# mynameisfiber/baton

Hardware: AMD Instinct MI355X
Metric: fed_local_samples_per_sec (higher is better)
Workload: dtype bf16; 1 GPU; model=resnet18, global_batch=8192, image=32x32x3, parallelism=federated-dp1 (FedAvg E=1), local_samples_per_round=16384, optimizer=sgd, hip_graph=True

## Files before the change

baton_amd/ops/csrc/bindings.cpp:

```cpp
#include <torch/extension.h>
#include <ATen/hip/HIPContext.h>

#include "launchers.h"
#include "wgrad_px_map.h"

namespace {

bool is_bf16(const at::Tensor& t) { return t.scalar_type() == at::kBFloat16; }

void check_compute(const at::Tensor& t, const char* name) {
  TORCH_CHECK(t.is_cuda(), name, " must be on GPU");
  TORCH_CHECK(t.is_contiguous(), name, " must be contiguous");
  TORCH_CHECK(t.scalar_type() == at::kFloat || t.scalar_type() == at::kBFloat16,
              name, " must be fp32 or bf16");
}

hipStream_t stream() { return at::hip::getCurrentHIPStream().stream(); }

void run_dense(const GemmProblem& p, const GemmPlan& pl, const void* A,
               const void* B, void* C, const float* bias, long long strideA = 0,
               long long strideB = 0, long long strideC = 0, int b_group = 1,
               GemmStrides gs = GemmStrides{0, 0, 0, 1, 0, 0, 0}) {
  if (pl.kind == GemmKind::G9) {
    TORCH_CHECK(launch_gemm_nt_g9(pl, A, B, C, bias, pl.m_main, p.N, p.K,
                                  (float)p.alpha, stream()),
                "gemm: G9 plan does not fit ", pl.m_main, "x", p.N, "x", p.K);
    if (pl.m_main == p.M) return;
    const GemmProblem r = gemm_remainder(p, pl);
    run_dense(r, plan_dense(r),
              (const at::BFloat16*)A + (long long)pl.m_main * p.K, B,
              (at::BFloat16*)C + (long long)pl.m_main * p.N, bias);
    return;
  }
  TORCH_CHECK(launch_gemm_2ph(pl, p, A, B, C, bias, strideA, strideB, strideC,
                              stream(), b_group, gs),
              "gemm: 2-phase plan does not fit ", p.M, "x", p.N, "x", p.K);
}

void run_slab(const GemmPlan& pl, const at::Tensor& A, const at::Tensor& B,
              at::Tensor& out, int M, int N, int K) {
  auto slabs = at::empty({(long long)pl.splits * M * N},
                         A.options().dtype(at::kFloat));
  TORCH_CHECK(launch_gemm_nt_slab(pl, A.data_ptr(), B.data_ptr(),
                                  slabs.data_ptr<float>(), out.data_ptr(),
                                  out.scalar_type() != at::kFloat, M, N, K,
                                  stream()),
              "gemm: slab plan does not fit ", M, "x", N, "x", K);
}

void run_splitk(const GemmPlan& pl, const at::Tensor& A, const at::Tensor& B,
                at::Tensor& out, int M, int N, int K) {
  TORCH_CHECK(launch_gemm_2ph_splitk(pl, is_bf16(A), A.data_ptr(), B.data_ptr(),
                                     out.data_ptr<float>(), M, N, K, stream()),
              "gemm: split-K plan does not fit ", M, "x", N, "x", K);
}

}


void sgd_step(at::Tensor p, at::Tensor g, at::Tensor m, double lr,
              double momentum, double weight_decay, bool zero_grad) {
  check_compute(p, "p");
  check_compute(g, "g");
  TORCH_CHECK(p.scalar_type() == g.scalar_type(), "p/g dtype mismatch");
  TORCH_CHECK(p.numel() == g.numel(), "p/g numel mismatch");
  float* mptr = nullptr;
  if (m.defined() && m.numel() > 0) {
    TORCH_CHECK(m.scalar_type() == at::kFloat && m.is_contiguous());
    TORCH_CHECK(m.numel() == p.numel());
    mptr = m.data_ptr<float>();
  }
  launch_sgd(is_bf16(p), p.data_ptr(), g.data_ptr(), mptr, p.numel(), (float)lr,
             (float)momentum, (float)weight_decay, zero_grad ? 1 : 0,
             stream());
}

void adam_step(at::Tensor p, at::Tensor g, at::Tensor m, at::Tensor v,
               double lr, double beta1, double beta2, double eps,
               double weight_decay, double bc1, double bc2, bool zero_grad) {
  check_compute(p, "p");
  check_compute(g, "g");
  TORCH_CHECK(m.scalar_type() == at::kFloat && v.scalar_type() == at::kFloat);
  TORCH_CHECK(p.numel() == g.numel() && p.numel() == m.numel() &&
              p.numel() == v.numel());
  launch_adam(is_bf16(p), p.data_ptr(), g.data_ptr(), m.data_ptr<float>(),
              v.data_ptr<float>(), p.numel(), (float)lr, (float)beta1,
              (float)beta2, (float)eps, (float)weight_decay,
// ... 464 lines not shown
      launch_conv_wgrad(is_bf16(x), dyt.data_ptr(), x.data_ptr(),
                        dw32.data_ptr(), N, H, W, Cin, Cout, (int)KH, (int)KW,
                        (int)stride, (int)pad, stream());
    }
  }
  if (out_f32 || x.scalar_type() == at::kFloat) return dw32;
  auto dw = at::empty({Cout, KH, KW, Cin}, x.options());
  launch_cast_copy(true, dw.data_ptr(), dw32.data_ptr<float>(), dw.numel(),
                   stream());
  return dw;
}


py::dict wgrad_px_map(int64_t N, int64_t H, int64_t W, int64_t step) {
  using namespace py::literals;
  TORCH_CHECK(wgpx::eligible(true, (int)N, (int)H, (int)W, 64, 64, 3, 3, 1, 1),
              "wgrad_px_map: shape not eligible");
  const wgpx::Geom g = wgpx::make_geom((int)H, (int)W);
  const long long p0 = step * wgpx::PXK;
  TORCH_CHECK(step >= 0 && p0 < N * H * W, "wgrad_px_map: step out of range");
  const int h0 = (int)((p0 / W) % H);
  const int passes = wgpx::passes_of((int)W);
  py::list stage, window, dy_rows;
  for (int i = 0; i < wgpx::PXK; ++i) dy_rows.append(py::none());
  for (int i = 0; i < g.slots; ++i) window.append(py::none());
  for (int c = 0; c < passes * wgpx::THREADS; ++c) {
    const wgpx::ChunkSrc cs = wgpx::chunk_src(g, c);
    const bool ok = cs.kind == 1 ||
                    (cs.kind == 2 && wgpx::x_row_valid(g, h0, cs.hrel));
    const long long px = ok ? p0 + cs.rel : -1;
    stage.append(py::make_tuple(c / wgpx::THREADS, c % wgpx::THREADS, 16 * c,
                                ok ? cs.kind : 0, px, cs.sub));
    const int row = c / wgpx::CPR;
    if (c % wgpx::CPR == 0 && row < wgpx::PXK) dy_rows[row] = cs.rel;
    if (c % wgpx::CPR == 0 && row >= wgpx::PXK && row < wgpx::PXK + g.slots &&
        ok)
      window[row - wgpx::PXK] = py::make_tuple(
          px / (H * W), (px / W) % H, px % W);
  }
  py::list kpix, a_addr, b_addr;
  for (int k = 0; k < wgpx::PXK; ++k)
    kpix.append(wgpx::lin_pixel((int)W, wgpx::kslot_lin(k)));
  for (int r = 0; r < 2; ++r) {
    py::list la;
    for (int l = 0; l < 64; ++l) la.append(wgpx::a_read_addr(l, r));
    a_addr.append(la);
  }
  for (int t = 0; t < 9; ++t) {
    py::list lt;
    for (int r = 0; r < 2; ++r) {
      py::list lb;
      for (int l = 0; l < 64; ++l)
        lb.append(wgpx::b_read_addr(g, l, r) +
                  wgpx::tap_off(g, t / 3, t % 3) * wgpx::ROWB);
      lt.append(lb);
    }
    b_addr.append(lt);
  }
  return py::dict(
      "row_bytes"_a = wgpx::ROWB, "dy_rows_base"_a = 0,
      "window_base"_a = wgpx::PXK * wgpx::ROWB, "pitch"_a = g.pitch,
      "window_rows"_a = g.wrows, "slots"_a = g.slots, "passes"_a = passes,
      "threads"_a = wgpx::THREADS, "buffer_bytes"_a = passes * wgpx::THREADS * 16,
      "claimed_conflict_degree"_a = 1, "stage"_a = stage, "window"_a = window,
      "dy_rows"_a = dy_rows, "kslot_pixel"_a = kpix, "a_addr"_a = a_addr,
      "b_addr"_a = b_addr);
}

bool wgrad_px_eligible(bool bf16, int64_t N, int64_t H, int64_t W, int64_t Cin,
                       int64_t Cout, int64_t KH, int64_t KW, int64_t stride,
                       int64_t pad) {
  return wgpx::eligible(bf16, (int)N, (int)H, (int)W, (int)Cin, (int)Cout,
                        (int)KH, (int)KW, (int)stride, (int)pad);
}

py::tuple wgrad_px_split(int64_t N, int64_t H, int64_t W, int64_t Cin,
                         int64_t Cout) {
  const long long steps = N * H * W / wgpx::PXK;
  const int sps = wgpx::steps_per_split(
      steps, (int)(Cin / wgpx::TILE) * (int)(Cout / wgpx::TILE));
  return py::make_tuple(steps, sps, (steps + sps - 1) / sps);
}


at::Tensor bmm_strided(at::Tensor A, at::Tensor B, c10::optional<at::Tensor> C_in,
                       int64_t layout, int64_t M, int64_t N, int64_t K,
                       int64_t nbatch, int64_t heads, int64_t b_group,
                       double alpha,
                       int64_t saO, int64_t saI, int64_t lda,
                       int64_t sbO, int64_t sbI, int64_t ldb,
                       int64_t scO, int64_t scI, int64_t ldc) {
  TORCH_CHECK(A.is_cuda() && B.is_cuda(), "bmm_strided: GPU tensors required");
  TORCH_CHECK(A.scalar_type() == B.scalar_type());
  TORCH_CHECK(A.scalar_type() == at::kFloat || A.scalar_type() == at::kBFloat16);
  at::Tensor C;
  if (C_in.has_value() && C_in->defined()) {
    C = *C_in;
    TORCH_CHECK(C.is_cuda() && C.scalar_type() == A.scalar_type());
  } else {
    C = at::empty({nbatch, M, N}, A.options());
    scO = (int64_t)heads * M * N;
    scI = (int64_t)M * N;
    ldc = N;
  }
  GemmStrides gs{lda, ldb, ldc, (int)heads, saI, sbI, scI};
  const GemmProblem p{is_bf16(A), false, (int)layout, (int)M, (int)N, (int)K,
                      false, false, alpha, 0.0, true, (int)nbatch,
                      gs.heads > 1 || gs.lda || gs.ldb || gs.ldc};
  run_dense(p, plan_dense(p), A.data_ptr(), B.data_ptr(), C.data_ptr(), nullptr,
            saO, sbO, scO, (int)b_group, gs);
  return C;
}


at::Tensor gemm_batched(at::Tensor A, at::Tensor B, int64_t layout,
                        bool out_f32, double alpha, int64_t b_group) {
  check_compute(A, "A");
  check_compute(B, "B");
  TORCH_CHECK(A.dim() == 3 && B.dim() == 3, "gemm_batched wants 3-D tensors");
  TORCH_CHECK(A.size(0) == B.size(0) * b_group, "batch/group mismatch");
  int nb = A.size(0);
  int M, N, K;
  if (layout == 0) {
    M = A.size(1); K = A.size(2); N = B.size(1);
    TORCH_CHECK(B.size(2) == K);
  } else if (layout == 1) {
    M = A.size(1); K = A.size(2); N = B.size(2);
    TORCH_CHECK(B.size(1) == K);
  } else {
    K = A.size(1); M = A.size(2); N = B.size(2);
    TORCH_CHECK(B.size(1) == K);
  }
  auto C = at::empty({nb, M, N},
                     A.options().dtype(out_f32 ? at::kFloat : A.scalar_type()));
  const GemmProblem p{is_bf16(A), out_f32, (int)layout, M, N, K, false, false,
                      alpha, 0.0, true, nb, false};
  run_dense(p, plan_dense(p), A.data_ptr(), B.data_ptr(), C.data_ptr(), nullptr,
            (long long)A.size(1) * A.size(2), (long long)B.size(1) * B.size(2),
            (long long)M * N, (int)b_group);
  return C;
}

at::Tensor softmax_fwd(at::Tensor x, double scale, int64_t causal_seq) {
  check_compute(x, "x");
  int C = x.size(-1);
  long long R = x.numel() / C;
  auto y = at::empty_like(x);
  launch_softmax_fwd(is_bf16(x), x.data_ptr(), y.data_ptr(), R, C,
                     (float)scale, (int)causal_seq, stream());
  return y;
}

at::Tensor softmax_bwd(at::Tensor y, at::Tensor dy, double scale) {
  check_compute(y, "y");
  check_compute(dy, "dy");
  int C = y.size(-1);
  long long R = y.numel() / C;
  auto dx = at::empty_like(y);
  launch_softmax_bwd(is_bf16(y), y.data_ptr(), dy.data_ptr(), dx.data_ptr(), R,
                     C, (float)scale, stream());
  return dx;
}



std::vector<at::Tensor> rms_fwd(at::Tensor x, at::Tensor w, double eps) {
// ... 178 lines not shown
      "flash_bwd_dq: unsupported head_dim ", DH);
  TORCH_CHECK(
      launch_flash_bwd_dkv(q.data_ptr(), k.data_ptr(), v.data_ptr(),
                           dout.data_ptr(), lse.data_ptr<float>(),
                           delta.data_ptr<float>(), dk.data_ptr(),
                           dv.data_ptr(), B, S, H, G, DH, scale, causal, qs,
                           ks, vs, dos, dks, dvs, stream()),
      "flash_bwd_dkv: unsupported head_dim ", DH);
}

PYBIND11_MODULE(TORCH_EXTENSION_NAME, m) {
  m.def("flash_fwd", &flash_fwd);
  m.def("flash_bwd", &flash_bwd);
  m.def("rms_add_fwd", &rms_add_fwd);
  m.def("rms_bwd_plus", &rms_bwd_plus);
  m.def("sgd_step", &sgd_step, "fused SGD step", py::arg("p"), py::arg("g"),
        py::arg("m"), py::arg("lr"), py::arg("momentum"),
        py::arg("weight_decay"), py::arg("zero_grad") = false);
  m.def("adam_step", &adam_step, "fused Adam step", py::arg("p"), py::arg("g"),
        py::arg("m"), py::arg("v"), py::arg("lr"), py::arg("beta1"),
        py::arg("beta2"), py::arg("eps"), py::arg("weight_decay"),
        py::arg("bc1"), py::arg("bc2"), py::arg("zero_grad") = false);
  m.def("scale_cast", &scale_cast);
  m.def("cast_copy", &cast_copy);
  m.def("axpby", &axpby);
  m.def("bmm_strided", &bmm_strided, py::arg("A"), py::arg("B"),
        py::arg("C_in") = py::none(), py::arg("layout") = 0,
        py::arg("M") = 0, py::arg("N") = 0, py::arg("K") = 0,
        py::arg("nbatch") = 1, py::arg("heads") = 1,
        py::arg("b_group") = 1, py::arg("alpha") = 1.0,
        py::arg("saO") = 0, py::arg("saI") = 0, py::arg("lda") = 0,
        py::arg("sbO") = 0, py::arg("sbI") = 0, py::arg("ldb") = 0,
        py::arg("scO") = 0, py::arg("scI") = 0, py::arg("ldc") = 0);
  m.def("colsum", &colsum);
  m.def("mse_fwd", &mse_fwd);
  m.def("mse_bwd", &mse_bwd);
  m.def("ce_fwd", &ce_fwd);
  m.def("ce_bwd", &ce_bwd);
  m.def("ln_fwd", &ln_fwd);
  m.def("ln_bwd", &ln_bwd);
  m.def("ln_add_fwd", &ln_add_fwd);
  m.def("ln_bwd_plus", &ln_bwd_plus);
  m.def("bn_fwd_train", &bn_fwd_train, py::arg("x"), py::arg("gamma"),
        py::arg("beta"), py::arg("running_mean"), py::arg("running_var"),
        py::arg("momentum"), py::arg("eps"), py::arg("relu"),
        py::arg("res") = py::none());
  m.def("bn_fwd_eval", &bn_fwd_eval);
  m.def("bn_bwd", &bn_bwd, py::arg("x"), py::arg("dy"), py::arg("y_post"),
        py::arg("mean"), py::arg("rstd"), py::arg("gamma"), py::arg("relu"),
        py::arg("want_dres") = false);
  m.def("relu_fwd", &relu_fwd);
  m.def("relu_bwd", &relu_bwd);
  m.def("add_relu_fwd", &add_relu_fwd);
  m.def("add_scaled_fwd", &add_scaled_fwd);
  m.def("scale_fwd", &scale_fwd);
  m.def("gelu_fwd", &gelu_fwd);
  m.def("gelu_bwd", &gelu_bwd);
  m.def("gemm", &gemm, py::arg("A"), py::arg("B"), py::arg("layout"),
        py::arg("bias") = py::none(), py::arg("relu") = false,
        py::arg("out_f32") = false, py::arg("alpha") = 1.0,
        py::arg("beta") = 0.0, py::arg("C_in") = py::none(),
        py::arg("direct") = false);
  m.def("gemm_plan", &gemm_plan, py::arg("M"), py::arg("N"), py::arg("K"),
        py::arg("layout") = 0, py::arg("bf16") = true,
        py::arg("out_f32") = false, py::arg("has_bias") = false,
        py::arg("relu") = false, py::arg("alpha") = 1.0, py::arg("beta") = 0.0,
        py::arg("direct") = false, py::arg("nbatch") = 1,
        py::arg("strided") = false, py::arg("batched") = false);
  m.def("gemm_batched", &gemm_batched, py::arg("A"), py::arg("B"),
        py::arg("layout"), py::arg("out_f32") = false, py::arg("alpha") = 1.0,
        py::arg("b_group") = 1);
  m.def("softmax_fwd", &softmax_fwd, py::arg("x"), py::arg("scale") = 1.0,
        py::arg("causal_seq") = 0);
  m.def("softmax_bwd", &softmax_bwd);
  m.def("rms_fwd", &rms_fwd);
  m.def("rms_bwd", &rms_bwd);
  m.def("rope", &rope, py::arg("x"), py::arg("cos_t"), py::arg("sin_t"),
        py::arg("inverse") = false);
  m.def("silu_mul_fwd", &silu_mul_fwd);
  m.def("silu_mul_bwd", &silu_mul_bwd);
  m.def("conv_fwd", &conv_fwd);
  m.def("conv_dgrad", &conv_dgrad);
  m.def("conv_wgrad", &conv_wgrad);
  m.def("wgrad_px_map", &wgrad_px_map, py::arg("N"), py::arg("H"),
        py::arg("W"), py::arg("step"));
  m.def("wgrad_px_eligible", &wgrad_px_eligible);
  m.def("wgrad_px_split", &wgrad_px_split);
}
```

baton_amd/ops/csrc/conv.hip:

```cpp
#include "common.h"

constexpr int CBK = 32;
constexpr int CFRAG = 16;

struct ConvShape {
  int N, H, W, Cin, Cout, KH, KW, stride, pad, HO, WO, swz;
};



template <int ROWS>
DEVINL void stage_glds_rows(bf16* __restrict__ lds, const bf16* __restrict__ src,
                            long long ld, long long row0, int k0) {
  const int t = threadIdx.x;
  const int w = t >> 6;
  constexpr int TOTAL = ROWS * 4;
#pragma unroll
  for (int p = 0; p * kBlock < TOTAL; ++p) {
    const int idx = p * kBlock + t;
    if (idx >= TOTAL) break;
    const int row = idx >> 2;
    const int psl = idx & 3;
    const int lsl = psl ^ ((row >> 2) & 3);
    auto g = (const __attribute__((address_space(1))) unsigned int*)(
        src + (row0 + row) * ld + k0 + lsl * 8);
    auto l = (__attribute__((address_space(3))) unsigned int*)(
        lds + (long long)(p * kBlock + w * 64) * 8);
    __builtin_amdgcn_global_load_lds(g, l, 16, 0, 0);
  }
}

template <typename T, int ROWS, bool FAST>
struct FwdAStager {
  static constexpr int ELEMS = 16 / (int)sizeof(T);
  static constexpr int TPR = CBK / ELEMS;
  static constexpr int RPP = kBlock / TPR;
  static constexpr int PASSES = ROWS / RPP;
  int kc;
  int row[PASSES];
  int n[PASSES], ho[PASSES], wo[PASSES];
  bool ok[PASSES];
  int ci, kw, kh;
  int k_generic;
  int m0_;
  bool full_;

  DEVINL void init(const ConvShape& sh, int m0, int Mtot) {
    m0_ = m0;
    full_ = (m0 + ROWS <= Mtot);
    kc = (threadIdx.x % TPR) * ELEMS;
#pragma unroll
    for (int p = 0; p < PASSES; ++p) {
      row[p] = p * RPP + threadIdx.x / TPR;
      const int m = m0 + row[p];
      wo[p] = m % sh.WO;
      const int t = m / sh.WO;
      ho[p] = t % sh.HO;
      n[p] = t / sh.HO;
      ok[p] = m < Mtot;
    }
    ci = kc;
    kw = 0;
    kh = 0;
    k_generic = kc;
  }

  DEVINL void stage(T* __restrict__ lds, const T* __restrict__ x,
                    const ConvShape& sh, int Ktot) {
    using VT = typename VecTraits<T>::VecT;
    if constexpr (sizeof(T) == 2 && FAST) {
      if (sh.KH == 1 && sh.stride == 1 && full_ && (sh.Cin % 8) == 0) {
        stage_glds_rows<ROWS>((bf16*)lds, (const bf16*)x, sh.Cin,
                              (long long)m0_, ci - kc);
        ci += CBK;
        if (ci >= sh.Cin) {
          ci -= sh.Cin;
          if (++kw == sh.KW) { kw = 0; ++kh; }
        }
        return;
      }
    }
#pragma unroll
    for (int p = 0; p < PASSES; ++p) {
// ... 68 lines not shown
                    ? w[(long long)(n0 + row) * ld + k0 + kc + j]
                    : (T)0.f;
    }
    *reinterpret_cast<VT*>(&lds[lds_off<T>(row, kc)]) = v;
  }
}

template <typename T, int ROWS, bool FAST>
struct DgradAStager {
  static constexpr int ELEMS = 16 / (int)sizeof(T);
  static constexpr int TPR = CBK / ELEMS;
  static constexpr int RPP = kBlock / TPR;
  static constexpr int PASSES = ROWS / RPP;
  int kc;
  int n[PASSES], hq[PASSES], wq[PASSES];
  bool ok[PASSES];
  int co, kw, kh;
  int k_generic;

  DEVINL void init(const ConvShape& sh, int m0, int Mtot) {
    kc = (threadIdx.x % TPR) * ELEMS;
#pragma unroll
    for (int p = 0; p < PASSES; ++p) {
      const int q = m0 + p * RPP + threadIdx.x / TPR;
      wq[p] = q % sh.W;
      const int t = q / sh.W;
      hq[p] = t % sh.H;
      n[p] = t / sh.H;
      ok[p] = q < Mtot;
    }
    co = kc;
    kw = 0;
    kh = 0;
    k_generic = kc;
  }

  DEVINL void stage(T* __restrict__ lds, const T* __restrict__ dy,
                    const ConvShape& sh, int Ktot) {
    using VT = typename VecTraits<T>::VecT;
#pragma unroll
    for (int p = 0; p < PASSES; ++p) {
      VT v;
      T* vp = reinterpret_cast<T*>(&v);
#pragma unroll
      for (int j = 0; j < ELEMS; ++j) vp[j] = (T)0.f;
      if (FAST) {
        if (ok[p]) {
          const int hnum = hq[p] + sh.pad - kh, wnum = wq[p] + sh.pad - kw;
          if (hnum >= 0 && wnum >= 0 && hnum % sh.stride == 0 &&
              wnum % sh.stride == 0) {
            const int ho = hnum / sh.stride, wo = wnum / sh.stride;
            if (ho < sh.HO && wo < sh.WO)
              v = *reinterpret_cast<const VT*>(
                  &dy[(((long long)n[p] * sh.HO + ho) * sh.WO + wo) * sh.Cout + co]);
          }
        }
      } else if (ok[p]) {
#pragma unroll
        for (int j = 0; j < ELEMS; ++j) {
          const int k = k_generic + j;
          if (k < Ktot) {
            const int coj = k % sh.Cout, tap = k / sh.Cout;
            const int kwj = tap % sh.KW, khj = tap / sh.KW;
            const int hnum = hq[p] + sh.pad - khj, wnum = wq[p] + sh.pad - kwj;
            if (hnum >= 0 && wnum >= 0 && hnum % sh.stride == 0 &&
                wnum % sh.stride == 0) {
              const int ho = hnum / sh.stride, wo = wnum / sh.stride;
              if (ho < sh.HO && wo < sh.WO)
                vp[j] = dy[(((long long)n[p] * sh.HO + ho) * sh.WO + wo) * sh.Cout + coj];
            }
          }
        }
      }
      *reinterpret_cast<VT*>(&lds[lds_off<T>(p * RPP + threadIdx.x / TPR, kc)]) = v;
    }
    if (FAST) {
      co += CBK;
      if (co >= sh.Cout) {
        co -= sh.Cout;
        if (++kw == sh.KW) { kw = 0; ++kh; }
      }
    } else {
      k_generic += CBK;
    }
  }
};

template <typename T, int ROWS>
struct WgradBStager {
  static constexpr int ELEMS = 16 / (int)sizeof(T);
  static constexpr int VPK = ROWS / ELEMS;
  static constexpr int TOTAL = CBK * VPK;
  static constexpr int PASSES = (TOTAL + kBlock - 1) / kBlock;
  int k_in_tile[PASSES], rr[PASSES], r_local[PASSES];
  int ci[PASSES], kw[PASSES], kh[PASSES];
  bool active[PASSES], one_tap[PASSES], r_ok[PASSES];
  int wo[PASSES], ho[PASSES], nn[PASSES];
  bool p_ok[PASSES];

  DEVINL void init(const ConvShape& sh, int n0, long long p0, long long p_limit,
                   int Rtot) {
#pragma unroll
    for (int p = 0; p < PASSES; ++p) {
      const int idx = p * kBlock + threadIdx.x;
      active[p] = idx < TOTAL;
      k_in_tile[p] = idx / VPK;
      r_local[p] = (idx % VPK) * ELEMS;
      rr[p] = n0 + r_local[p];
      r_ok[p] = rr[p] < Rtot;
      ci[p] = r_ok[p] ? rr[p] % sh.Cin : 0;
      const int tap = r_ok[p] ? rr[p] / sh.Cin : 0;
      kw[p] = tap % sh.KW;
      kh[p] = tap / sh.KW;
      one_tap[p] = (rr[p] / sh.Cin) == ((rr[p] + ELEMS - 1) / sh.Cin);
      const long long px = p0 + k_in_tile[p];
      p_ok[p] = px < p_limit;
      wo[p] = (int)(px % sh.WO);
      const long long t = px / sh.WO;
      ho[p] = (int)(t % sh.HO);
      nn[p] = (int)(t / sh.HO);
    }
  }

  DEVINL void stage(T* __restrict__ lds, const T* __restrict__ x,
                    const ConvShape& sh) {
    using VT = typename VecTraits<T>::VecT;
#pragma unroll
    for (int p = 0; p < PASSES; ++p) {
      if (!active[p]) continue;
      VT v;
      T* vp = reinterpret_cast<T*>(&v);
#pragma unroll
      for (int j = 0; j < ELEMS; ++j) vp[j] = (T)0.f;
      if (p_ok[p] && r_ok[p]) {
        if (one_tap[p]) {
          const int hi = ho[p] * sh.stride - sh.pad + kh[p];
          const int wi = wo[p] * sh.stride - sh.pad + kw[p];
          if (hi >= 0 && hi < sh.H && wi >= 0 && wi < sh.W)
            v = *reinterpret_cast<const VT*>(
                &x[(((long long)nn[p] * sh.H + hi) * sh.W + wi) * sh.Cin + ci[p]]);
        } else {
#pragma unroll
          for (int j = 0; j < ELEMS; ++j) {
            const int rj = rr[p] + j;
            const int cij = rj % sh.Cin, tapj = rj / sh.Cin;
            const int kwj = tapj % sh.KW, khj = tapj / sh.KW;
            const int hi = ho[p] * sh.stride - sh.pad + khj;
            const int wi = wo[p] * sh.stride - sh.pad + kwj;
            if (hi >= 0 && hi < sh.H && wi >= 0 && wi < sh.W)
              vp[j] = x[(((long long)nn[p] * sh.H + hi) * sh.W + wi) * sh.Cin + cij];
          }
        }
      }
#pragma unroll
      for (int j = 0; j < ELEMS; ++j)
        lds[lds_off<T>(r_local[p] + j, k_in_tile[p])] = vp[j];
      wo[p] += CBK;
      while (wo[p] >= sh.WO) {
        wo[p] -= sh.WO;
        if (++ho[p] == sh.HO) { ho[p] = 0; ++nn[p]; }
      }
    }
  }

  DEVINL void set_p_ok(long long p0, long long p_limit) {
#pragma unroll
// ... 75 lines not shown
  FwdAStager<T, BM, FAST> sa;
  sa.init(sh, m0, Mtot);
  sa.stage(a_lds[0], x, sh, Ktot);
  stage_fwd_B<T, BN>(b_lds[0], w, n0, 0, Ntot, Ktot, Ktot);
  __syncthreads();
  for (int kt = 0; kt < nk; ++kt) {
    const int cur = kt & 1;
    if (kt + 1 < nk) {
      sa.stage(a_lds[cur ^ 1], x, sh, Ktot);
      stage_fwd_B<T, BN>(b_lds[cur ^ 1], w, n0, (kt + 1) * CBK, Ntot, Ktot, Ktot);
    }
    conv_mma<T, MF, NF>(a_lds[cur], b_lds[cur], acc, lane, wm0, wn0);
    __syncthreads();
  }
  const int col_in_frag = lane & 15, row_base = (lane >> 4) * 4;
#pragma unroll
  for (int mf = 0; mf < MF; ++mf)
#pragma unroll
    for (int nf = 0; nf < NF; ++nf)
#pragma unroll
      for (int r = 0; r < 4; ++r) {
        int row = m0 + wm0 + mf * CFRAG + row_base + r;
        int col = n0 + wn0 + nf * CFRAG + col_in_frag;
        if (row < Mtot && col < Ntot)
          y[(long long)row * Ntot + col] = (T)acc[mf][nf][r];
      }
}

template <typename T, int BM, int BN, int WAVES_M, int WAVES_N, bool FAST>
__global__ __launch_bounds__(kBlock) void conv_dgrad_kernel(
    const T* __restrict__ dy, const T* __restrict__ w_t, T* __restrict__ dx,
    ConvShape sh) {
  constexpr int WM = BM / WAVES_M, WN = BN / WAVES_N;
  constexpr int MF = WM / CFRAG, NF = WN / CFRAG;
  __shared__ T a_lds[2][BM * lds_row_elems<T>()];
  __shared__ T b_lds[2][BN * lds_row_elems<T>()];
  const int Mtot = sh.N * sh.H * sh.W;
  const int Ntot = sh.Cin;
  const int Ktot = sh.KH * sh.KW * sh.Cout;
  int t_n, t_m;
  {
    const int nwg = gridDim.x * gridDim.y;
    int bid = blockIdx.y * gridDim.x + blockIdx.x;
    if (sh.swz && nwg >= 64) {
      const int q = nwg >> 3, r = nwg & 7;
      const int xcd = bid & 7, idx = bid >> 3;
      bid = (xcd < r ? xcd * (q + 1) : r * (q + 1) + (xcd - r) * q) + idx;
    }
    t_n = bid % gridDim.x;
    t_m = bid / gridDim.x;
  }
  const int m0 = t_m * BM, n0 = t_n * BN;
  const int lane = threadIdx.x & (kWave - 1);
  const int wid = threadIdx.x / kWave;
  const int wm0 = (wid / WAVES_N) * WM, wn0 = (wid % WAVES_N) * WN;
  f32x4 acc[MF][NF] = {};
  const int nk = (Ktot + CBK - 1) / CBK;
  DgradAStager<T, BM, FAST> sa;
  sa.init(sh, m0, Mtot);
  sa.stage(a_lds[0], dy, sh, Ktot);
  stage_fwd_B<T, BN>(b_lds[0], w_t, n0, 0, Ntot, Ktot, Ktot);
  __syncthreads();
  for (int kt = 0; kt < nk; ++kt) {
    const int cur = kt & 1;
    if (kt + 1 < nk) {
      sa.stage(a_lds[cur ^ 1], dy, sh, Ktot);
      stage_fwd_B<T, BN>(b_lds[cur ^ 1], w_t, n0, (kt + 1) * CBK, Ntot, Ktot, Ktot);
    }
    conv_mma<T, MF, NF>(a_lds[cur], b_lds[cur], acc, lane, wm0, wn0);
    __syncthreads();
  }
  const int col_in_frag = lane & 15, row_base = (lane >> 4) * 4;
#pragma unroll
  for (int mf = 0; mf < MF; ++mf)
#pragma unroll
    for (int nf = 0; nf < NF; ++nf)
#pragma unroll
      for (int r = 0; r < 4; ++r) {
        int row = m0 + wm0 + mf * CFRAG + row_base + r;
        int col = n0 + wn0 + nf * CFRAG + col_in_frag;
        if (row < Mtot && col < Ntot)
          dx[(long long)row * Ntot + col] = (T)acc[mf][nf][r];
      }
}

template <typename T, int BM, int BN, int WAVES_M, int WAVES_N>
__global__ __launch_bounds__(kBlock) void conv_wgrad_kernel(
    const T* __restrict__ dy_t, const T* __restrict__ x, float* __restrict__ dw,
    ConvShape sh, long long p_chunk) {
  constexpr int WM = BM / WAVES_M, WN = BN / WAVES_N;
  constexpr int MF = WM / CFRAG, NF = WN / CFRAG;
  __shared__ T a_lds[2][BM * lds_row_elems<T>()];
  __shared__ T b_lds[2][BN * lds_row_elems<T>()];
  const int Mtot = sh.Cout;
  const int Ntot = sh.KH * sh.KW * sh.Cin;
  const long long Ptot = (long long)sh.N * sh.HO * sh.WO;
  const long long p_begin = (long long)blockIdx.z * p_chunk;
  const long long p_end = min(p_begin + p_chunk, Ptot);
  const int m0 = blockIdx.y * BM, n0 = blockIdx.x * BN;
  const int lane = threadIdx.x & (kWave - 1);
  const int wid = threadIdx.x / kWave;
  const int wm0 = (wid / WAVES_N) * WM, wn0 = (wid % WAVES_N) * WN;
  f32x4 acc[MF][NF] = {};
  const long long nk = (p_end - p_begin + CBK - 1) / CBK;
  if (nk <= 0) return;
  WgradBStager<T, BN> sb;
  sb.init(sh, n0, p_begin, p_end, Ntot);
  stage_fwd_B<T, BM>(a_lds[0], dy_t, m0, (int)p_begin, Mtot, (int)p_end, Ptot);
  sb.stage(b_lds[0], x, sh);
  __syncthreads();
  for (long long kt = 0; kt < nk; ++kt) {
    const int cur = (int)(kt & 1);
    if (kt + 1 < nk) {
      stage_fwd_B<T, BM>(a_lds[cur ^ 1], dy_t, m0,
                         (int)(p_begin + (kt + 1) * CBK), Mtot, (int)p_end,
                         Ptot);
      sb.set_p_ok(p_begin + (kt + 1) * CBK, p_end);
      sb.stage(b_lds[cur ^ 1], x, sh);
    }
    conv_mma<T, MF, NF>(a_lds[cur], b_lds[cur], acc, lane, wm0, wn0);
    __syncthreads();
  }
  const int col_in_frag = lane & 15, row_base = (lane >> 4) * 4;
#pragma unroll
  for (int mf = 0; mf < MF; ++mf)
#pragma unroll
    for (int nf = 0; nf < NF; ++nf)
#pragma unroll
      for (int r = 0; r < 4; ++r) {
        int row = m0 + wm0 + mf * CFRAG + row_base + r;
        int col = n0 + wn0 + nf * CFRAG + col_in_frag;
        if (row < Mtot && col < Ntot) {
          if (gridDim.z == 1)
            dw[(long long)row * Ntot + col] = acc[mf][nf][r];
          else
            atomicAdd(&dw[(long long)row * Ntot + col], acc[mf][nf][r]);
        }
      }
}

#define INST_CONV(T)                                                        \
  template __global__ void conv_fwd_kernel<T, 128, 128, 2, 2, true>(        \
      const T*, const T*, T*, ConvShape);                                   \
  template __global__ void conv_fwd_kernel<T, 128, 128, 2, 2, false>(       \
      const T*, const T*, T*, ConvShape);                                   \
  template __global__ void conv_fwd_kernel<T, 128, 64, 4, 1, true>(         \
      const T*, const T*, T*, ConvShape);                                   \
  template __global__ void conv_fwd_kernel<T, 128, 64, 4, 1, false>(        \
      const T*, const T*, T*, ConvShape);                                   \
  template __global__ void conv_dgrad_kernel<T, 128, 128, 2, 2, true>(      \
      const T*, const T*, T*, ConvShape);                                   \
  template __global__ void conv_dgrad_kernel<T, 128, 128, 2, 2, false>(     \
      const T*, const T*, T*, ConvShape);                                   \
  template __global__ void conv_dgrad_kernel<T, 128, 64, 4, 1, true>(       \
      const T*, const T*, T*, ConvShape);                                   \
  template __global__ void conv_dgrad_kernel<T, 128, 64, 4, 1, false>(      \
      const T*, const T*, T*, ConvShape);                                   \
  template __global__ void conv_wgrad_kernel<T, 128, 128, 2, 2>(            \
      const T*, const T*, float*, ConvShape, long long);                    \
  template __global__ void conv_wgrad_kernel<T, 64, 128, 1, 4>(             \
      const T*, const T*, float*, ConvShape, long long);

INST_CONV(bf16)
INST_CONV(float)

#include "launchers.h"

static ConvShape make_shape(int N, int H, int W, int Cin, int Cout, int KH,
                            int KW, int stride, int pad) {
  ConvShape sh;
  sh.N = N; sh.H = H; sh.W = W; sh.Cin = Cin; sh.Cout = Cout;
  sh.KH = KH; sh.KW = KW; sh.stride = stride; sh.pad = pad;
  sh.HO = (H + 2 * pad - KH) / stride + 1;
  sh.WO = (W + 2 * pad - KW) / stride + 1;
  long long act = (long long)N * H * W * Cin + (long long)N * sh.HO * sh.WO * Cout;
  sh.swz = act * 2 > (200LL << 20) ? 1 : 0;
  return sh;
}

void launch_conv_fwd(bool is_bf16, const void* x, const void* w, void* y,
                     int N, int H, int W, int Cin, int Cout, int KH, int KW,
                     int stride, int pad, hipStream_t s) {
  ConvShape sh = make_shape(N, H, W, Cin, Cout, KH, KW, stride, pad);
  long long M = (long long)N * sh.HO * sh.WO;
  const bool narrow = Cout <= 64;
  const bool fast = (Cin % CBK) == 0;
  const int BN_ = narrow ? 64 : 128;
  dim3 grid((Cout + BN_ - 1) / BN_, (M + 127) / 128);
  #define FWD(T, BM, BN, WM, WN, F)                                         \
    hipLaunchKernelGGL((conv_fwd_kernel<T, BM, BN, WM, WN, F>), grid,       \
                       dim3(kBlock), 0, s, (const T*)x, (const T*)w, (T*)y, sh)
  if (is_bf16) {
    if (narrow) { if (fast) FWD(bf16, 128, 64, 4, 1, true); else FWD(bf16, 128, 64, 4, 1, false); }
    else { if (fast) FWD(bf16, 128, 128, 2, 2, true); else FWD(bf16, 128, 128, 2, 2, false); }
  } else {
    if (narrow) { if (fast) FWD(float, 128, 64, 4, 1, true); else FWD(float, 128, 64, 4, 1, false); }
    else { if (fast) FWD(float, 128, 128, 2, 2, true); else FWD(float, 128, 128, 2, 2, false); }
  }
  #undef FWD
}

void launch_conv_dgrad(bool is_bf16, const void* dy, const void* w, void* dx,
                       int N, int H, int W, int Cin, int Cout, int KH, int KW,
                       int stride, int pad, hipStream_t s) {
  ConvShape sh = make_shape(N, H, W, Cin, Cout, KH, KW, stride, pad);
  long long M = (long long)N * H * W;
  const bool narrow = Cin <= 64;
  const bool fast = (Cout % CBK) == 0;
  const int BN_ = narrow ? 64 : 128;
  dim3 grid((Cin + BN_ - 1) / BN_, (M + 127) / 128);
  #define DG(T, BM, BN, WM, WN, F)                                          \
    hipLaunchKernelGGL((conv_dgrad_kernel<T, BM, BN, WM, WN, F>), grid,     \
                       dim3(kBlock), 0, s, (const T*)dy, (const T*)w, (T*)dx, sh)
  if (is_bf16) {
    if (narrow) { if (fast) DG(bf16, 128, 64, 4, 1, true); else DG(bf16, 128, 64, 4, 1, false); }
    else { if (fast) DG(bf16, 128, 128, 2, 2, true); else DG(bf16, 128, 128, 2, 2, false); }
  } else {
    if (narrow) { if (fast) DG(float, 128, 64, 4, 1, true); else DG(float, 128, 64, 4, 1, false); }
    else { if (fast) DG(float, 128, 128, 2, 2, true); else DG(float, 128, 128, 2, 2, false); }
  }
  #undef DG
}

void launch_conv_wgrad(bool is_bf16, const void* dy, const void* x, void* dw,
                       int N, int H, int W, int Cin, int Cout, int KH, int KW,
                       int stride, int pad, hipStream_t s) {
  ConvShape sh = make_shape(N, H, W, Cin, Cout, KH, KW, stride, pad);
  int Ntot = KH * KW * Cin;
  const bool narrow_m = Cout <= 64;
  const int BM_ = narrow_m ? 64 : 128;
  int tiles_x = (Ntot + 127) / 128;
  int tiles_y = (Cout + BM_ - 1) / BM_;
  long long Ptot = (long long)N * sh.HO * sh.WO;
  int target = 512 / (tiles_x * tiles_y);
  if (target < 1) target = 1;
  long long max_splits = (Ptot + CBK - 1) / CBK;
  int splits = (int)(max_splits < target ? max_splits : target);
  long long p_chunk = ((Ptot + splits - 1) / splits + CBK - 1) / CBK * CBK;
  splits = (int)((Ptot + p_chunk - 1) / p_chunk);
  dim3 grid(tiles_x, tiles_y, splits);
  #define WG(T, BM, BN, WM, WN)                                             \
    hipLaunchKernelGGL((conv_wgrad_kernel<T, BM, BN, WM, WN>), grid,        \
                       dim3(kBlock), 0, s, (const T*)dy, (const T*)x,       \
                       (float*)dw, sh, p_chunk)
  if (is_bf16) { if (narrow_m) WG(bf16, 64, 128, 1, 4); else WG(bf16, 128, 128, 2, 2); }
  else { if (narrow_m) WG(float, 64, 128, 1, 4); else WG(float, 128, 128, 2, 2); }
  #undef WG
}
```

baton_amd/ops/functional.py:

```python

from __future__ import annotations

import os
from typing import Optional

import torch
import torch.nn.functional as F

from baton_amd.ops._ext import require_hip


def _on_gpu(*tensors: torch.Tensor) -> bool:
    return tensors[0].is_cuda


_LIB_GEMM = os.environ.get("BATON_LIB_GEMM", "1") != "0"


def _lib_gemm(x: torch.Tensor) -> bool:
    return _LIB_GEMM and x.dtype == torch.bfloat16


def lib_gemm_enabled() -> bool:
    return _LIB_GEMM
# ... 1 lines not shown

class LinearFn(torch.autograd.Function):

    @staticmethod
    def forward(ctx, x, weight, bias, weight_t=None):
        ctx.save_for_backward(x, weight, weight_t)
        ctx.has_bias = bias is not None
        if _on_gpu(x):
            if _lib_gemm(x):
                if bias is None:
                    return x @ weight.t()
                return torch.addmm(bias.to(x.dtype), x, weight.t())
            ops = require_hip()
            return ops.gemm(x, weight, 0, bias, False, False, 1.0, 0.0)
        out = x @ weight.t()
        if bias is not None:
            out = out + bias.to(out.dtype)
        return out

    @staticmethod
    def backward(ctx, dy):
        x, weight, weight_t = ctx.saved_tensors
        dy = dy.contiguous()
        need_dx, need_dw, need_db = ctx.needs_input_grad[:3]
        dx = dw = db = None
        if _on_gpu(dy):
            ops = require_hip()
            if need_dx:
                if _lib_gemm(dy):
                    dx = dy @ weight
                elif weight_t is not None:
                    dx = ops.gemm(dy, weight_t, 0)
                else:
                    dx = ops.gemm(dy, weight, 1)
            if need_dw:
                if _lib_gemm(dy):
                    dw = (dy.t() @ x).to(weight.dtype)
                elif dy.shape[1] <= 32:
                    dw = ops.gemm(dy.t().contiguous(), x, 1, None, False,
                                  False, 1.0, 0.0, None, True)
                    dw = dw.to(weight.dtype)
                else:
                    dw = ops.gemm(dy, x, 2).to(weight.dtype)
            if need_db and ctx.has_bias:
                db = ops.colsum(dy)
        else:
            if need_dx:
                dx = dy @ weight
            if need_dw:
                dw = (dy.t() @ x).to(weight.dtype)
            if need_db and ctx.has_bias:
                db = dy.sum(0, dtype=torch.float32)
        return dx, dw, db, None


def linear(x: torch.Tensor, weight: torch.Tensor,
           bias: Optional[torch.Tensor] = None,
           weight_t: Optional[torch.Tensor] = None):
    shape = x.shape
    x2 = x.reshape(-1, shape[-1]).contiguous()
    y = LinearFn.apply(x2, weight, bias, weight_t)
    return y.reshape(*shape[:-1], weight.shape[0])


class Conv2dFn(torch.autograd.Function):

    @staticmethod
    def forward(ctx, x, w, stride: int, pad: int):
        ctx.save_for_backward(x, w)
        ctx.stride, ctx.pad = stride, pad
        if _on_gpu(x):
            ops = require_hip()
            return ops.conv_fwd(x, w, stride, pad)
        xn = x.permute(0, 3, 1, 2)
        wn = w.permute(0, 3, 1, 2)
        y = F.conv2d(xn.float(), wn.float(), stride=stride, padding=pad)
        return y.permute(0, 2, 3, 1).contiguous().to(x.dtype)

    @staticmethod
    def backward(ctx, dy):
        x, w = ctx.saved_tensors
        stride, pad = ctx.stride, ctx.pad
        dy = dy.contiguous()
        if _on_gpu(dy):
            ops = require_hip()
            dx = ops.conv_dgrad(dy, w, x.shape[1], x.shape[2], stride, pad)
            dw = ops.conv_wgrad(dy, x, w.shape[1], w.shape[2], stride, pad, False)
        else:
            xn = x.permute(0, 3, 1, 2).float()
            wn = w.permute(0, 3, 1, 2).float()
            dyn = dy.permute(0, 3, 1, 2).float()
            dxn = torch.nn.grad.conv2d_input(xn.shape, wn, dyn, stride=stride, padding=pad)
            dwn = torch.nn.grad.conv2d_weight(xn, wn.shape, dyn, stride=stride, padding=pad)
            dx = dxn.permute(0, 2, 3, 1).contiguous().to(x.dtype)
            dw = dwn.permute(0, 2, 3, 1).contiguous().to(w.dtype)
        return dx, dw, None, None


def conv2d(x, w, stride: int = 1, pad: int = 0):
    return Conv2dFn.apply(x, w, stride, pad)


class LayerNormFn(torch.autograd.Function):
    @staticmethod
    def forward(ctx, x, weight, bias, eps: float):
        x = x.contiguous()
        if _on_gpu(x):
            ops = require_hip()
            y, mean, rstd = ops.ln_fwd(x, weight, bias, eps)
        else:
            C = x.shape[-1]
            xf = x.float().reshape(-1, C)
            mean = xf.mean(dim=1)
            var = xf.var(dim=1, unbiased=False)
            rstd = (var + eps).rsqrt()
            y = ((xf - mean[:, None]) * rstd[:, None] * weight.float() +
                 bias.float()).to(x.dtype).reshape(x.shape)
        ctx.save_for_backward(x, weight, mean, rstd)
        return y

    @staticmethod
    def backward(ctx, dy):
        x, weight, mean, rstd = ctx.saved_tensors
        dy = dy.contiguous()
        if _on_gpu(dy):
            ops = require_hip()
            dx, dw, db = ops.ln_bwd(x, dy, weight, mean, rstd)
        else:
            C = x.shape[-1]
            xf = x.float().reshape(-1, C)
            dyf = dy.float().reshape(-1, C)
            xhat = (xf - mean[:, None]) * rstd[:, None]
            dyg = dyf * weight.float()
            m1 = dyg.mean(dim=1, keepdim=True)
            m2 = (dyg * xhat).mean(dim=1, keepdim=True)
            dx = (rstd[:, None] * (dyg - m1 - xhat * m2)).to(x.dtype).reshape(x.shape)
            dw = (dyf * xhat).sum(0)
            db = dyf.sum(0)
        return dx, dw.to(weight.dtype), db.to(weight.dtype), None


def layer_norm(x, weight, bias, eps: float = 1e-5):
    return LayerNormFn.apply(x, weight, bias, eps)


class LayerNormAddFn(torch.autograd.Function):

    @staticmethod
    def forward(ctx, x, res, weight, bias, eps: float):
        x = x.contiguous()
        res = res.contiguous()
        if _on_gpu(x):
            ops = require_hip()
            y, z, mean, rstd = ops.ln_add_fwd(x, res, weight, bias, eps)
        else:
            z = (x.float() + res.float()).to(x.dtype)
            C = x.shape[-1]
            zf = z.float().reshape(-1, C)
            mean = zf.mean(dim=1)
            var = zf.var(dim=1, unbiased=False)
            rstd = (var + eps).rsqrt()
            y = ((zf - mean[:, None]) * rstd[:, None] * weight.float() +
                 bias.float()).to(x.dtype).reshape(x.shape)
        ctx.save_for_backward(z, weight, mean, rstd)
        return y

    @staticmethod
    def backward(ctx, dy):
        z, weight, mean, rstd = ctx.saved_tensors
        dy = dy.contiguous()
        if _on_gpu(dy):
            dz, dw, db = require_hip().ln_bwd(z, dy, weight, mean, rstd)
        else:
            C = z.shape[-1]
            zf = z.float().reshape(-1, C)
            dyf = dy.float().reshape(-1, C)
            xhat = (zf - mean[:, None]) * rstd[:, None]
            dyg = dyf * weight.float()
# ... 789 lines not shown
```

Measured before the change: 103,800 samples/s.

## Add phase-decomposed dgrad kernel for stride-2 convs and skip unneeded grads

Adds a sub-pixel phase decomposition for stride-2 conv dgrad. Output pixels are grouped into four parity classes, and each class iterates only over the kernel taps that actually contribute, so the implicit GEMM no longer loops over taps that fail the stride divisibility test. A host-built map of classes and tiles is passed to a new kernel that scatters results back through a per-row pixel table. Separately, conv backward now skips dx or dw when autograd does not need them, such as dx for the first conv on the input images. The new path adds tile-to-class lookup and an indirect store pattern.

```diff
diff --git a/baton_amd/ops/csrc/bindings.cpp b/baton_amd/ops/csrc/bindings.cpp
--- a/baton_amd/ops/csrc/bindings.cpp
+++ b/baton_amd/ops/csrc/bindings.cpp
@@ -3,6 +3,7 @@
 
 #include "launchers.h"
 #include "wgrad_px_map.h"
+#include "dgrad_phase_map.h"
 
 namespace {
 
@@ -633,6 +634,44 @@
   return py::make_tuple(steps, sps, (steps + sps - 1) / sps);
 }
 
+
+py::dict dgrad_phase_map(int64_t N, int64_t H, int64_t W, int64_t KH,
+                         int64_t KW, int64_t stride, int64_t pad, int64_t BM,
+                         int64_t n_tiles, bool swz) {
+  using namespace py::literals;
+  TORCH_CHECK(N > 0 && H > 0 && W > 0 && BM > 0 && n_tiles > 0 &&
+                  dgph::eligible((int)N, (int)H, (int)W, 32, (int)KH, (int)KW,
+                                 (int)stride, (int)pad, 32),
+              "dgrad_phase_map: shape not eligible");
+  const dgph::Map m = dgph::make_map((int)N, (int)H, (int)W, (int)KH, (int)KW,
+                                     (int)pad, (int)BM);
+  py::list classes;
+  for (int i = 0; i < dgph::NCLS; ++i) {
+    const dgph::Class& c = m.cls[i];
+    py::list taps, rows;
+    for (int t = c.tap0; t < c.tap0 + c.ntaps; ++t)
+      taps.append(py::make_tuple((int)m.taps[t].kh, (int)m.taps[t].kw,
+                                 (int)m.taps[t].dh, (int)m.taps[t].dw));
+    for (int r = 0; r < c.rows; ++r) {
+      const dgph::RowPos p = dgph::row_pos(c, r);
+      const int px = dgph::row_pixel(m, c, r);
+      TORCH_CHECK(px == (p.n * (int)H + 2 * p.a + c.ph) * (int)W + 2 * p.b + c.pw);
+      rows.append(py::make_tuple(px / (int)(H * W), (px / (int)W) % (int)H,
+                                 px % (int)W));
+    }
+    classes.append(py::dict("ph"_a = c.ph, "pw"_a = c.pw, "Hc"_a = c.Hc,
+                            "Wc"_a = c.Wc, "rows"_a = rows, "n_rows"_a = c.rows,
+                            "tile0"_a = c.tile0, "tiles"_a = c.tiles,
+                            "taps"_a = taps));
+  }
+  py::list blocks;
+  for (int b = 0; b < m.m_tiles * (int)n_tiles; ++b) {
+    const dgph::Tile t = dgph::block_tile(m, b, (int)n_tiles, swz ? 1 : 0);
+    blocks.append(py::make_tuple(t.cls, t.m_tile, t.n_tile));
+  }
+  return py::dict("BM"_a = m.BM, "m_tiles"_a = m.m_tiles, "classes"_a = classes,
+                  "blocks"_a = blocks);
+}
 
 at::Tensor bmm_strided(at::Tensor A, at::Tensor B, c10::optional<at::Tensor> C_in,
                        int64_t layout, int64_t M, int64_t N, int64_t K,
@@ -977,6 +1016,10 @@
   m.def("conv_fwd", &conv_fwd);
   m.def("conv_dgrad", &conv_dgrad);
   m.def("conv_wgrad", &conv_wgrad);
+  m.def("dgrad_phase_map", &dgrad_phase_map, py::arg("N"), py::arg("H"),
+        py::arg("W"), py::arg("KH"), py::arg("KW"), py::arg("stride"),
+        py::arg("pad"), py::arg("BM"), py::arg("n_tiles") = 1,
+        py::arg("swz") = false);
   m.def("wgrad_px_map", &wgrad_px_map, py::arg("N"), py::arg("H"),
         py::arg("W"), py::arg("step"));
   m.def("wgrad_px_eligible", &wgrad_px_eligible);
diff --git a/baton_amd/ops/csrc/conv.hip b/baton_amd/ops/csrc/conv.hip
--- a/baton_amd/ops/csrc/conv.hip
+++ b/baton_amd/ops/csrc/conv.hip
@@ -1,4 +1,5 @@
 #include "common.h"
+#include "dgrad_phase_map.h"
 
 constexpr int CBK = 32;
 constexpr int CFRAG = 16;
@@ -233,6 +234,45 @@
       }
     } else {
       k_generic += CBK;
+    }
+  }
+};
+
+template <typename T, int ROWS>
+struct DgradPhaseAStager {
+  static constexpr int ELEMS = 16 / (int)sizeof(T);
+  static constexpr int TPR = CBK / ELEMS;
+  static constexpr int RPP = kBlock / TPR;
+  static constexpr int PASSES = ROWS / RPP;
+  int kc;
+  int n[PASSES], a[PASSES], b[PASSES];
+  bool ok[PASSES];
+
+  DEVINL void init(const dgph::Class& c, int r0) {
+    kc = (threadIdx.x % TPR) * ELEMS;
+#pragma unroll
+    for (int p = 0; p < PASSES; ++p) {
+      const int r = r0 + p * RPP + threadIdx.x / TPR;
+      const dgph::RowPos pos = dgph::row_pos(c, r);
+      n[p] = pos.n; a[p] = pos.a; b[p] = pos.b;
+      ok[p] = r < c.rows;
+    }
+  }
+
+  DEVINL void stage(T* __restrict__ lds, const T* __restrict__ dy,
+                    const ConvShape& sh, int dh, int dw, int co0) {
+    using VT = typename VecTraits<T>::VecT;
+#pragma unroll
+    for (int p = 0; p < PASSES; ++p) {
+      VT v;
+      T* vp = reinterpret_cast<T*>(&v);
+#pragma unroll
+      for (int j = 0; j < ELEMS; ++j) vp[j] = (T)0.f;
+      const int ho = a[p] + dh, wo = b[p] + dw;
+      if (ok[p] && ho >= 0 && ho < sh.HO && wo >= 0 && wo < sh.WO)
+        v = *reinterpret_cast<const VT*>(
+            &dy[(((long long)n[p] * sh.HO + ho) * sh.WO + wo) * sh.Cout + co0 + kc]);
+      *reinterpret_cast<VT*>(&lds[lds_off<T>(p * RPP + threadIdx.x / TPR, kc)]) = v;
     }
   }
 };
@@ -474,6 +514,65 @@
         if (row < Mtot && col < Ntot)
           dx[(long long)row * Ntot + col] = (T)acc[mf][nf][r];
       }
+}
+
+template <typename T, int BM, int BN, int WAVES_M, int WAVES_N>
+__global__ __launch_bounds__(kBlock) void conv_dgrad_phase_kernel(
+    const T* __restrict__ dy, const T* __restrict__ w_t, T* __restrict__ dx,
+    ConvShape sh, dgph::Map mp) {
+  constexpr int WM = BM / WAVES_M, WN = BN / WAVES_N;
+  constexpr int MF = WM / CFRAG, NF = WN / CFRAG;
+  static_assert(BM <= kBlock, "one thread per row fills row_px");
+  __shared__ T a_lds[2][BM * lds_row_elems<T>()];
+  __shared__ T b_lds[2][BN * lds_row_elems<T>()];
+  __shared__ int row_px[BM];
+  const int Ntot = sh.Cin;
+  const int Ktot = sh.KH * sh.KW * sh.Cout;
+  const int n_tiles = (Ntot + BN - 1) / BN;
+  const dgph::Tile tile = dgph::block_tile(mp, blockIdx.x, n_tiles, sh.swz);
+  const dgph::Class& cls = mp.cls[tile.cls];
+  const int r0 = tile.m_tile * BM, n0 = tile.n_tile * BN;
+  const int lane = threadIdx.x & (kWave - 1);
+  const int wid = threadIdx.x / kWave;
+  const int wm0 = (wid / WAVES_N) * WM, wn0 = (wid % WAVES_N) * WN;
+  f32x4 acc[MF][NF] = {};
+  const int nk = cls.ntaps * (sh.Cout / CBK);
+  if (threadIdx.x < BM) {
+    const int r = r0 + threadIdx.x;
+    row_px[threadIdx.x] = r < cls.rows ? dgph::row_pixel(mp, cls, r) : -1;
+  }
+  DgradPhaseAStager<T, BM> sa;
+  sa.init(cls, r0);
+  int tap = cls.tap0, co0 = 0;
+  auto stage = [&](int buf) {
+    const dgph::Tap tp = mp.taps[tap];
+    sa.stage(a_lds[buf], dy, sh, tp.dh, tp.dw, co0);
+    stage_fwd_B<T, BN>(b_lds[buf], w_t, n0,
+                       (tp.kh * sh.KW + tp.kw) * sh.Cout + co0, Ntot, Ktot, Ktot);
+    co0 += CBK;
+    if (co0 == sh.Cout) { co0 = 0; ++tap; }
+  };
+  if (nk > 0) stage(0);
+  __syncthreads();
+  for (int kt = 0; kt < nk; ++kt) {
+    const int cur = kt & 1;
+    if (kt + 1 < nk) stage(cur ^ 1);
+    conv_mma<T, MF, NF>(a_lds[cur], b_lds[cur], acc, lane, wm0, wn0);
+    __syncthreads();
+  }
+  const int col_in_frag = lane & 15, row_base = (lane >> 4) * 4;
+#pragma unroll
+  for (int mf = 0; mf < MF; ++mf)
+#pragma unroll
+    for (int r = 0; r < 4; ++r) {
+      const int px = row_px[wm0 + mf * CFRAG + row_base + r];
+      if (px < 0) continue;
+#pragma unroll
+      for (int nf = 0; nf < NF; ++nf) {
+        const int col = n0 + wn0 + nf * CFRAG + col_in_frag;
+        if (col < Ntot) dx[(long long)px * Ntot + col] = (T)acc[mf][nf][r];
+      }
+    }
 }
 
 template <typename T, int BM, int BN, int WAVES_M, int WAVES_N>
@@ -548,6 +647,10 @@
       const T*, const T*, T*, ConvShape);                                   \
   template __global__ void conv_dgrad_kernel<T, 128, 64, 4, 1, false>(      \
       const T*, const T*, T*, ConvShape);                                   \
+  template __global__ void conv_dgrad_phase_kernel<T, 128, 128, 2, 2>(      \
+      const T*, const T*, T*, ConvShape, dgph::Map);                        \
+  template __global__ void conv_dgrad_phase_kernel<T, 128, 64, 4, 1>(       \
+      const T*, const T*, T*, ConvShape, dgph::Map);                        \
   template __global__ void conv_wgrad_kernel<T, 128, 128, 2, 2>(            \
       const T*, const T*, float*, ConvShape, long long);                    \
   template __global__ void conv_wgrad_kernel<T, 64, 128, 1, 4>(             \
@@ -600,6 +703,18 @@
   const bool narrow = Cin <= 64;
   const bool fast = (Cout % CBK) == 0;
   const int BN_ = narrow ? 64 : 128;
+  if (dgph::eligible(N, H, W, Cout, KH, KW, stride, pad, CBK)) {
+    const dgph::Map mp = dgph::make_map(N, H, W, KH, KW, pad, 128);
+    dim3 pgrid((unsigned)(mp.m_tiles * ((Cin + BN_ - 1) / BN_)));
+    #define DGP(T, BM, BN, WM, WN)                                          \
+      hipLaunchKernelGGL((conv_dgrad_phase_kernel<T, BM, BN, WM, WN>),      \
+                         pgrid, dim3(kBlock), 0, s, (const T*)dy,           \
+                         (const T*)w, (T*)dx, sh, mp)
+    if (is_bf16) { if (narrow) DGP(bf16, 128, 64, 4, 1); else DGP(bf16, 128, 128, 2, 2); }
+    else { if (narrow) DGP(float, 128, 64, 4, 1); else DGP(float, 128, 128, 2, 2); }
+    #undef DGP
+    return;
+  }
   dim3 grid((Cin + BN_ - 1) / BN_, (M + 127) / 128);
   #define DG(T, BM, BN, WM, WN, F)                                          \
     hipLaunchKernelGGL((conv_dgrad_kernel<T, BM, BN, WM, WN, F>), grid,     \
diff --git a/baton_amd/ops/csrc/dgrad_phase_map.h b/baton_amd/ops/csrc/dgrad_phase_map.h
--- /dev/null
+++ b/baton_amd/ops/csrc/dgrad_phase_map.h
@@ -0,0 +1,123 @@
+#pragma once
+
+#if defined(__HIPCC__)
+#define DGPH_HD __host__ __device__ inline
+#else
+#define DGPH_HD inline
+#endif
+
+namespace dgph {
+
+constexpr int STRIDE = 2;
+constexpr int NCLS = STRIDE * STRIDE;
+constexpr int MAX_TAPS = 49;
+
+struct Tap {
+  signed char kh, kw;
+  signed char dh, dw;
+};
+
+struct Class {
+  int ph, pw;
+  int Hc, Wc;
+  int rows;
+  int tile0, tiles;
+  int tap0, ntaps;
+};
+
+struct Map {
+  int N, H, W, BM;
+  int m_tiles;
+  Class cls[NCLS];
+  Tap taps[MAX_TAPS];
+};
+
+DGPH_HD bool eligible(int N, int H, int W, int Cout, int KH, int KW,
+                      int stride, int pad, int cbk) {
+  if (stride != STRIDE || Cout % cbk != 0) return false;
+  if (KH < 1 || KW < 1 || KH * KW > MAX_TAPS || pad < 0 || pad > 63)
+    return false;
+  return (long long)N * H * W < (1LL << 31) - 4096;
+}
+
+DGPH_HD int axis_taps(int p, int pad, int K) {
+  const int k0 = (p + pad) % STRIDE;
+  return K > k0 ? (K - k0 + STRIDE - 1) / STRIDE : 0;
+}
+
+DGPH_HD Map make_map(int N, int H, int W, int KH, int KW, int pad, int BM) {
+  Map m{};
+  m.N = N; m.H = H; m.W = W; m.BM = BM;
+  int order[NCLS], count[NCLS];
+  for (int c = 0; c < NCLS; ++c) {
+    order[c] = c;
+    count[c] = axis_taps(c / STRIDE, pad, KH) * axis_taps(c % STRIDE, pad, KW);
+  }
+  for (int i = 1; i < NCLS; ++i)
+    for (int j = i; j > 0 && count[order[j]] > count[order[j - 1]]; --j) {
+      const int t = order[j]; order[j] = order[j - 1]; order[j - 1] = t;
+    }
+  int tile = 0, tap = 0;
+  for (int i = 0; i < NCLS; ++i) {
+    Class& c = m.cls[i];
+    c.ph = order[i] / STRIDE;
+    c.pw = order[i] % STRIDE;
+    c.Hc = H > c.ph ? (H - c.ph + STRIDE - 1) / STRIDE : 0;
+    c.Wc = W > c.pw ? (W - c.pw + STRIDE - 1) / STRIDE : 0;
+    c.rows = N * c.Hc * c.Wc;
+    c.tile0 = tile;
+    c.tiles = (c.rows + BM - 1) / BM;
+    tile += c.tiles;
+    c.tap0 = tap;
+    for (int kh = 0; kh < KH; ++kh) {
+      const int hn = c.ph + pad - kh;
+      if (hn % STRIDE != 0) continue;
+      for (int kw = 0; kw < KW; ++kw) {
+        const int wn = c.pw + pad - kw;
+        if (wn % STRIDE != 0) continue;
+        Tap& t = m.taps[tap++];
+        t.kh = (signed char)kh; t.kw = (signed char)kw;
+        t.dh = (signed char)(hn / STRIDE); t.dw = (signed char)(wn / STRIDE);
+      }
+    }
+    c.ntaps = tap - c.tap0;
+  }
+  m.m_tiles = tile;
+  return m;
+}
+
+struct RowPos { int n, a, b; };
+DGPH_HD RowPos row_pos(const Class& c, int r) {
+  RowPos p;
+  p.b = r % c.Wc;
+  const int t = r / c.Wc;
+  p.a = t % c.Hc;
+  p.n = t / c.Hc;
+  return p;
+}
+
+DGPH_HD int row_pixel(const Map& m, const Class& c, int r) {
+  const RowPos p = row_pos(c, r);
+  return (p.n * m.H + STRIDE * p.a + c.ph) * m.W + STRIDE * p.b + c.pw;
+}
+
+struct Tile { int cls, m_tile, n_tile; };
+DGPH_HD Tile block_tile(const Map& m, int bid, int n_tiles, int swz) {
+  int c = 0;
+  for (int i = 1; i < NCLS; ++i)
+    if (bid >= m.cls[i].tile0 * n_tiles) c = i;
+  int local = bid - m.cls[c].tile0 * n_tiles;
+  const int nwg = m.cls[c].tiles * n_tiles;
+  if (swz && nwg >= 64) {
+    const int q = nwg >> 3, r = nwg & 7;
+    const int xcd = local & 7, idx = local >> 3;
+    local = (xcd < r ? xcd * (q + 1) : r * (q + 1) + (xcd - r) * q) + idx;
+  }
+  Tile t;
+  t.cls = c;
+  t.n_tile = local % n_tiles;
+  t.m_tile = local / n_tiles;
+  return t;
+}
+
+}
diff --git a/baton_amd/ops/functional.py b/baton_amd/ops/functional.py
--- a/baton_amd/ops/functional.py
+++ b/baton_amd/ops/functional.py
@@ -107,18 +107,24 @@
         x, w = ctx.saved_tensors
         stride, pad = ctx.stride, ctx.pad
         dy = dy.contiguous()
-        if _on_gpu(dy):
-            ops = require_hip()
-            dx = ops.conv_dgrad(dy, w, x.shape[1], x.shape[2], stride, pad)
-            dw = ops.conv_wgrad(dy, x, w.shape[1], w.shape[2], stride, pad, False)
+        need_dx, need_dw = ctx.needs_input_grad[:2]
+        dx = dw = None
+        if _on_gpu(dy):
+            ops = require_hip()
+            if need_dx:
+                dx = ops.conv_dgrad(dy, w, x.shape[1], x.shape[2], stride, pad)
+            if need_dw:
+                dw = ops.conv_wgrad(dy, x, w.shape[1], w.shape[2], stride, pad, False)
         else:
             xn = x.permute(0, 3, 1, 2).float()
             wn = w.permute(0, 3, 1, 2).float()
             dyn = dy.permute(0, 3, 1, 2).float()
-            dxn = torch.nn.grad.conv2d_input(xn.shape, wn, dyn, stride=stride, padding=pad)
-            dwn = torch.nn.grad.conv2d_weight(xn, wn.shape, dyn, stride=stride, padding=pad)
-            dx = dxn.permute(0, 2, 3, 1).contiguous().to(x.dtype)
-            dw = dwn.permute(0, 2, 3, 1).contiguous().to(w.dtype)
+            if need_dx:
+                dxn = torch.nn.grad.conv2d_input(xn.shape, wn, dyn, stride=stride, padding=pad)
+                dx = dxn.permute(0, 2, 3, 1).contiguous().to(x.dtype)
+            if need_dw:
+                dwn = torch.nn.grad.conv2d_weight(xn, wn.shape, dyn, stride=stride, padding=pad)
+                dw = dwn.permute(0, 2, 3, 1).contiguous().to(w.dtype)
         return dx, dw, None, None
 
 
```

After: 114,600 samples/s, median of 6. 10.4% higher.
